# zhouxian/act3d-chained-diffuser

Measured on AMD Instinct MI355X. Metric: train samples/sec (Act3D keypose fwd+bwd+AdamW step), higher is better.
Workload: dtype fp16 / bf16 MFMA on two-part operands (x = hi + lo; fp32 accumulate) in attention; fp32-accurate linears (f32 MFMA; bf16x3 MFMA from 4096 rows); bf16 frozen backbone + FPN; 1 GPU; Act3D keypose training step, 18-PerAct-task shapes: 4 cameras 256x256, 3 ghost-point levels, 1000 ghost points (333/level), E=60, frozen synthetic CLIP-RN50-shaped backbone + trainable FPN included in the step; per_gpu_batch_keyframes=64, global_batch=64, parallelism=dp1, hipgraph=True, backbone_prefetch=True

## Files before the change

act3d-chained-diffuser_amd/csrc/conv1x1_deep.hip:

```cpp
#include "a3d_common.h"
#include "../../include/act3d_hip.h"

namespace a3d {

constexpr int CD_BM = 128, CD_BN = 128, CD_BK = 64;

__device__ __forceinline__ int cd_xoff(int row, int seg) { return row * 64 + ((seg ^ ((row >> 1) & 7)) << 3); }
__device__ __forceinline__ int cd_woff(int row, int seg) { return row * 64 + ((seg ^ ((((row >> 4) & 3) << 1) | ((row >> 1) & 1))) << 3); }

__device__ __forceinline__ unsigned int cd_norm2(unsigned int u, const float* scS, int K, int k, float relu_lo) {
  float a = __uint_as_float(u << 16) * scS[k] + scS[K + k];
  float b = __uint_as_float(u & 0xFFFF0000u) * scS[k + 1] + scS[K + k + 1];
  return pk_bf16(fmaxf(a, relu_lo), fmaxf(b, relu_lo));
}

__device__ __forceinline__ void cd_compute(const unsigned short* Xb, const unsigned short* Wb, const int (&xo)[2][4], const int (&wo)[2][4],
                                           f32x4 (&acc)[4][4]) {
#pragma unroll
  for (int h = 0; h < 2; ++h) {
    s16x8 xa[4], wb[4];
#pragma unroll
    for (int i = 0; i < 4; ++i) {
      xa[i] = *reinterpret_cast<const s16x8*>(&Xb[xo[h][i]]);
      wb[i] = *reinterpret_cast<const s16x8*>(&Wb[wo[h][i]]);
    }
#pragma unroll
    for (int tn = 0; tn < 4; ++tn)
#pragma unroll
      for (int tm = 0; tm < 4; ++tm) acc[tn][tm] = mfma_bf16_16x16x32(wb[tn], xa[tm], acc[tn][tm]);
  }
}

__device__ __forceinline__ void cd_epilogue(f32x4 (&acc)[4][4], float (&ssum)[4][4], float (&ssq)[4][4], unsigned short* __restrict__ y,
                                            long long m0, long long M, int N, int n0, int wm, int wn, int li, int g) {
#pragma unroll
  for (int tm = 0; tm < 4; ++tm) {
    const long long m = m0 + wm * 64 + tm * 16 + li;
    const bool ok = m < M;
    unsigned int pk[8];
#pragma unroll
    for (int tn = 0; tn < 4; ++tn) {
#pragma unroll
      for (int r2 = 0; r2 < 2; ++r2) {
        const unsigned int u = pk_bf16(acc[tn][tm][2 * r2], acc[tn][tm][2 * r2 + 1]);
        const float v0 = ok ? __uint_as_float(u << 16) : 0.f, v1 = ok ? __uint_as_float(u & 0xFFFF0000u) : 0.f;
        ssum[tn][2 * r2] += v0;
        ssq[tn][2 * r2] += v0 * v0;
        ssum[tn][2 * r2 + 1] += v1;
        ssq[tn][2 * r2 + 1] += v1 * v1;
        pk[2 * tn + r2] = u;
      }
      acc[tn][tm] = f32x4{0.f, 0.f, 0.f, 0.f};
    }
    if (ok) {
      uint4* dst = reinterpret_cast<uint4*>(y + (size_t)m * N + n0 + wn * 64 + g * 16);
      dst[0] = make_uint4(pk[0], pk[1], pk[2], pk[3]);
      dst[1] = make_uint4(pk[4], pk[5], pk[6], pk[7]);
    }
  }
}

template <bool XFORM>
__global__ __launch_bounds__(256, 2) void conv1x1_deep_kernel(const unsigned short* __restrict__ x, const unsigned short* __restrict__ w,
                                                            const float* __restrict__ in_scale, const float* __restrict__ in_shift,
                                                            int in_relu, unsigned short* __restrict__ y, float* __restrict__ partial,
                                                            long long M, int N, int K) {
  extern __shared__ __attribute__((aligned(16))) unsigned short smem_cd[];
  unsigned short* Xs = smem_cd;
  unsigned short* Ws = Xs + 2 * CD_BM * CD_BK;
  float* scS = reinterpret_cast<float*>(Ws + 2 * CD_BN * CD_BK);
  const int t = threadIdx.x, lane = t & 63, wave = t >> 6;
  const int li = lane & 15, g = lane >> 4;
  const int wm = wave >> 1, wn = wave & 1;
  const int n0 = blockIdx.y * CD_BN;
  const int KS = K / CD_BK;
  const long long mtiles = (M + CD_BM - 1) / CD_BM;
  if (XFORM)
    for (int i = t; i < K; i += 256) { scS[i] = in_scale[i]; scS[K + i] = in_shift[i]; }
  float ssum[4][4], ssq[4][4];
#pragma unroll
  for (int a = 0; a < 4; ++a)
#pragma unroll
    for (int r = 0; r < 4; ++r) { ssum[a][r] = 0.f; ssq[a][r] = 0.f; }
  const long long my_tiles = blockIdx.x < mtiles ? (mtiles - blockIdx.x + gridDim.x - 1) / gridDim.x : 0;
  const long long total = my_tiles * KS;
  const int srow = t >> 3, sseg = t & 7;
  long long l_m0 = (long long)blockIdx.x * CD_BM;
  int l_ks = 0;
  const float relu_lo = in_relu ? 0.f : -INFINITY;
#define CD_LOAD1(P, i)                                                                                                \
  {                                                                                                                   \
    const long long m_ = l_m0 + srow + 32 * i < M ? l_m0 + srow + 32 * i : M - 1;    \
    P##x##i = *reinterpret_cast<const uint4*>(x + (size_t)m_ * K + l_ks * CD_BK + sseg * 8);                          \
    P##w##i = *reinterpret_cast<const uint4*>(w + (size_t)(n0 + srow + 32 * i) * K + l_ks * CD_BK + sseg * 8);        \
  }
#define CD_LOAD(P)                                                                                                    \
  do {                                                                                                                \
    CD_LOAD1(P, 0) CD_LOAD1(P, 1) CD_LOAD1(P, 2) CD_LOAD1(P, 3)                                                       \
    if (l_left > 1) { --l_left; if (++l_ks == KS) { l_ks = 0; l_m0 += (long long)gridDim.x * CD_BM; } }               \
  } while (0)
#define CD_STAGE1(P, i)                                                                                               \
  {                                                                                                                   \
    uint4 v = P##x##i;                                                                                                \
    if (XFORM) {                                                                                                      \
      const int k0 = ks * CD_BK + sseg * 8;                                                                           \
      unsigned int u0 = v.x, u1 = v.y, u2 = v.z, u3 = v.w;                                                            \
      u0 = cd_norm2(u0, scS, K, k0 + 0, relu_lo); u1 = cd_norm2(u1, scS, K, k0 + 2, relu_lo);                         \
      u2 = cd_norm2(u2, scS, K, k0 + 4, relu_lo); u3 = cd_norm2(u3, scS, K, k0 + 6, relu_lo);                         \
      v = make_uint4(u0, u1, u2, u3);                                                                                 \
    }                                                                                                                 \
    *reinterpret_cast<uint4*>(&Xs[buf * CD_BM * CD_BK + cd_xoff(srow + 32 * i, sseg)]) = v;                           \
    *reinterpret_cast<uint4*>(&Ws[buf * CD_BN * CD_BK + cd_woff(srow + 32 * i, sseg)]) = P##w##i;                     \
  }
#define CD_STAGE(P) CD_STAGE1(P, 0) CD_STAGE1(P, 1) CD_STAGE1(P, 2) CD_STAGE1(P, 3)
  int xo[2][4], wo[2][4];
#pragma unroll
  for (int h = 0; h < 2; ++h)
#pragma unroll
    for (int i = 0; i < 4; ++i) {
      xo[h][i] = cd_xoff(wm * 64 + i * 16 + li, h * 4 + g);
      wo[h][i] = cd_woff(wn * 64 + (li >> 2) * 16 + i * 4 + (li & 3), h * 4 + g);
    }
  if (total > 0) {
    uint4 ax0, ax1, ax2, ax3, aw0, aw1, aw2, aw3, bx0, bx1, bx2, bx3, bw0, bw1, bw2, bw3;
    long long l_left = total;
    CD_LOAD(a);
    CD_LOAD(b);
    long long c_m0 = (long long)blockIdx.x * CD_BM;
    int ks = 0;
    f32x4 acc[4][4];
#pragma unroll
    for (int a = 0; a < 4; ++a)
#pragma unroll
      for (int b = 0; b < 4; ++b) acc[a][b] = f32x4{0.f, 0.f, 0.f, 0.f};
    __syncthreads();
#define CD_STEP(P, BUF)                                                                                               \
    {                                                                                                                 \
      constexpr int buf = BUF;                                                                                        \
      CD_STAGE(P)                                                                                                     \
      CD_LOAD(P);                                                                                \
      __syncthreads();                                             \
      cd_compute(Xs + buf * CD_BM * CD_BK, Ws + buf * CD_BN * CD_BK, xo, wo, acc);                                    \
      if (ks == KS - 1) cd_epilogue(acc, ssum, ssq, y, c_m0, M, N, n0, wm, wn, li, g);                                \
      if (++ks == KS) { ks = 0; c_m0 += (long long)gridDim.x * CD_BM; }                                               \
    }
    for (long long s = 0; s < total; s += 2) {
      CD_STEP(a, 0)
      if (s + 1 < total) CD_STEP(b, 1)
    }
#undef CD_STEP
  }
  if (!partial) return;
  __syncthreads();
  float* redS = reinterpret_cast<float*>(Xs);
  float* redQ = redS + 4 * 64;
#pragma unroll
  for (int tn = 0; tn < 4; ++tn)
#pragma unroll
    for (int r = 0; r < 4; ++r) {
      float sv = ssum[tn][r], q = ssq[tn][r];
#pragma unroll
      for (int o = 1; o < 16; o <<= 1) { sv += __shfl_xor(sv, o, 64); q += __shfl_xor(q, o, 64); }
      if (li == 0) { redS[wave * 64 + g * 16 + tn * 4 + r] = sv; redQ[wave * 64 + g * 16 + tn * 4 + r] = q; }
    }
  __syncthreads();
  if (t < CD_BN) {
    const int wn_i = t >> 6, c = t & 63;
    const float sv = redS[(0 * 2 + wn_i) * 64 + c] + redS[(1 * 2 + wn_i) * 64 + c];
    const float q = redQ[(0 * 2 + wn_i) * 64 + c] + redQ[(1 * 2 + wn_i) * 64 + c];
    float* p = partial + (size_t)blockIdx.x * 2 * N;
    p[n0 + t] = sv;
    p[N + n0 + t] = q;
  }
}

#undef CD_LOAD
#undef CD_LOAD1
#undef CD_STAGE1
#undef CD_STAGE

}

using namespace a3d;

bool a3d::conv1x1_deep_serves(int K, int N) { return K >= 128 && K <= 2048 && (K % CD_BK) == 0 && N >= 128 && N <= 2048 && (N % CD_BN) == 0; }
static size_t cd_lds(int K, bool xform) { return (size_t)2 * (CD_BM + CD_BN) * CD_BK * 2 + (xform ? (size_t)2 * K * sizeof(float) : 0); }

int a3d::conv1x1_deep_slabs(size_t M, int K, int N) {
  (void)K;
  const size_t mtiles = (M + CD_BM - 1) / CD_BM;
  const int nblocks = N / CD_BN;
  return (int)std::min<size_t>(mtiles, (size_t)std::max(1, 512 / nblocks));
}

int a3d::conv1x1_deep_launch(const void* x, const void* w, const float* in_scale, const float* in_shift, int in_relu, void* y, float* partial,
                             size_t M, int K, int N, hipStream_t s) {
  if (in_scale && K > 1024) { set_error("a3d_conv1x1_bn_fwd: the folded BatchNorm-apply of the deep-layer kernel serves K <= 1024 (K=%d)", K); return A3D_ERR_ARG; }
  static bool once = false;
  if (!once) {
    (void)hipFuncSetAttribute((const void*)conv1x1_deep_kernel<false>, hipFuncAttributeMaxDynamicSharedMemorySize, 80 * 1024);
    (void)hipFuncSetAttribute((const void*)conv1x1_deep_kernel<true>, hipFuncAttributeMaxDynamicSharedMemorySize, 80 * 1024);
    once = true;
  }
  const dim3 grid(conv1x1_deep_slabs(M, K, N), N / CD_BN);
  if (in_scale)
    hipLaunchKernelGGL(conv1x1_deep_kernel<true>, grid, dim3(256), cd_lds(K, true), s, (const unsigned short*)x, (const unsigned short*)w,
                       in_scale, in_shift, in_relu, (unsigned short*)y, partial, (long long)M, N, K);
  else
    hipLaunchKernelGGL(conv1x1_deep_kernel<false>, grid, dim3(256), cd_lds(K, false), s, (const unsigned short*)x, (const unsigned short*)w,
                       in_scale, in_shift, in_relu, (unsigned short*)y, partial, (long long)M, N, K);
  return check_launch("a3d_conv1x1_bn_fwd(deep)");
}
```

Baseline: 3476 samples/s.

## Replace deep conv1x1 kernel with 3-stage direct-to-LDS pipelined persistent GEMM

Adds a new deep-layer 1x1 conv GEMM that stages X and W tiles through a three-deep LDS ring using global_load_lds with explicit vmcnt waits, with BM selectable as 128 or 256 rows, XCD-aware persistent tile scheduling, and split partial BatchNorm-statistics output. The aim is to hide global-memory latency behind MFMA work and to improve L2 locality on MI355X. The old kernel is kept as a legacy path behind an environment variable. The change raises LDS use and drops to one workgroup per CU, and its hand-written inline asm and wait-count logic could be fragile.

```diff
diff --git a/act3d-chained-diffuser_amd/csrc/conv1x1_deep.hip b/act3d-chained-diffuser_amd/csrc/conv1x1_deep.hip
--- a/act3d-chained-diffuser_amd/csrc/conv1x1_deep.hip
+++ b/act3d-chained-diffuser_amd/csrc/conv1x1_deep.hip
@@ -1,4 +1,5 @@
 #include "a3d_common.h"
+#include "attn_ring.h"
 #include "../../include/act3d_hip.h"
 
 namespace a3d {
@@ -61,7 +62,7 @@
 }
 
 template <bool XFORM>
-__global__ __launch_bounds__(256, 2) void conv1x1_deep_kernel(const unsigned short* __restrict__ x, const unsigned short* __restrict__ w,
+__global__ __launch_bounds__(256, 2) void conv1x1_deep_legacy_kernel(const unsigned short* __restrict__ x, const unsigned short* __restrict__ w,
                                                             const float* __restrict__ in_scale, const float* __restrict__ in_shift,
                                                             int in_relu, unsigned short* __restrict__ y, float* __restrict__ partial,
                                                             long long M, int N, int K) {
@@ -179,12 +180,261 @@
 #undef CD_STAGE1
 #undef CD_STAGE
 
+
+constexpr int CR_BN = 128, CR_BK = 64, CR_STAGES = 3;
+
+template <int N_>
+__device__ __forceinline__ void cr_wait_vm() { asm volatile("s_waitcnt vmcnt(%0)" ::"n"(N_) : "memory"); }
+__device__ __forceinline__ void cr_store16(void* p, u32x4_ v) { asm volatile("global_store_dwordx4 %0, %1, off\n\ts_nop 1" ::"v"(p), "v"(v) : "memory"); }
+__device__ __forceinline__ void cr_glds16_dep(const void* g, void* lds, int& dep) {
+  const unsigned int dst = __builtin_amdgcn_readfirstlane((unsigned int)(size_t)(lds_void_t*)lds);
+  asm volatile("s_mov_b32 m0, %2\n\ts_nop 0\n\tglobal_load_lds_dwordx4 %1, off" : "+v"(dep) : "v"(g), "s"(dst) : "memory", "m0");
+}
+
+template <int TM>
+__device__ __forceinline__ void cr_compute(const unsigned short* xp0, const unsigned short* xp1, const unsigned short* wp0,
+                                           const unsigned short* wp1, f32x4 (&acc)[4][TM]) {
+#pragma unroll
+  for (int h = 0; h < 2; ++h) {
+    const unsigned short* xp = h ? xp1 : xp0;
+    const unsigned short* wp = h ? wp1 : wp0;
+    s16x8 xa[TM], wb[4];
+#pragma unroll
+    for (int i = 0; i < 4; ++i) wb[i] = *reinterpret_cast<const s16x8*>(wp + i * 4 * CR_BK);
+#pragma unroll
+    for (int i = 0; i < TM; ++i) xa[i] = *reinterpret_cast<const s16x8*>(xp + i * 16 * CR_BK);
+#pragma unroll
+    for (int tn = 0; tn < 4; ++tn)
+#pragma unroll
+      for (int tm = 0; tm < TM; ++tm) acc[tn][tm] = mfma_bf16_16x16x32(wb[tn], xa[tm], acc[tn][tm]);
+  }
+}
+
+template <int TM, bool COUNTED>
+__device__ __forceinline__ void cr_epilogue(f32x4 (&acc)[4][TM], float (&ssum)[4][4], float (&ssq)[4][4], unsigned short* __restrict__ y,
+                                            long long m0, long long M, int N, int n0, int wm, int wn, int li, int g) {
+#pragma unroll
+  for (int tm = 0; tm < TM; ++tm) {
+    const long long m = m0 + wm * (16 * TM) + tm * 16 + li;
+    const bool ok = COUNTED || m < M;
+    unsigned int pk[8];
+#pragma unroll
+    for (int tn = 0; tn < 4; ++tn) {
+#pragma unroll
+      for (int r2 = 0; r2 < 2; ++r2) {
+        const unsigned int u = pk_bf16(acc[tn][tm][2 * r2], acc[tn][tm][2 * r2 + 1]);
+        const float v0 = ok ? __uint_as_float(u << 16) : 0.f, v1 = ok ? __uint_as_float(u & 0xFFFF0000u) : 0.f;
+        ssum[tn][2 * r2] += v0;
+        ssq[tn][2 * r2] += v0 * v0;
+        ssum[tn][2 * r2 + 1] += v1;
+        ssq[tn][2 * r2 + 1] += v1 * v1;
+        pk[2 * tn + r2] = u;
+      }
+      acc[tn][tm] = f32x4{0.f, 0.f, 0.f, 0.f};
+    }
+    unsigned short* dst = y + (size_t)m * N + n0 + wn * 64 + g * 16;
+    if (COUNTED) {
+      cr_store16(dst, u32x4_{pk[0], pk[1], pk[2], pk[3]});
+      cr_store16(dst + 8, u32x4_{pk[4], pk[5], pk[6], pk[7]});
+    } else if (ok) {
+      reinterpret_cast<uint4*>(dst)[0] = make_uint4(pk[0], pk[1], pk[2], pk[3]);
+      reinterpret_cast<uint4*>(dst)[1] = make_uint4(pk[4], pk[5], pk[6], pk[7]);
+    }
+  }
+}
+
+template <bool XFORM, int TM>
+__global__ __launch_bounds__(256, 1) void conv1x1_deep_kernel(const unsigned short* __restrict__ x, const unsigned short* __restrict__ w,
+                                                            const float* __restrict__ in_scale, const float* __restrict__ in_shift,
+                                                            int in_relu, unsigned short* __restrict__ y, float* __restrict__ partial,
+                                                            long long M, int N, int K, int ngroups, int nslab) {
+  constexpr int BM = 32 * TM;
+  constexpr int STAGE = (BM + CR_BN) * CR_BK;
+  constexpr int NDMA = XFORM ? 4 : TM + 4;
+  extern __shared__ __attribute__((aligned(16))) unsigned short smem_cr[];
+  float* scS = reinterpret_cast<float*>(smem_cr + CR_STAGES * STAGE);
+  int slab, nb;
+  if (!xcd_decode(N / CR_BN, ngroups, slab, nb)) return;
+  const int t = threadIdx.x, lane = t & 63, wave = t >> 6;
+  const int li = lane & 15, g = lane >> 4;
+  const int wm = wave >> 1, wn = wave & 1;
+  const int n0 = nb * CR_BN;
+  const int KS = K / CR_BK;
+  const long long mtiles = (M + BM - 1) / BM;
+  const long long my_tiles = (mtiles - slab + ngroups - 1) / ngroups;
+  const long long total = my_tiles * KS;
+  const long long tile_stride = (long long)ngroups * BM;
+  if (XFORM) {
+    for (int i = t; i < K; i += 256) { scS[i] = in_scale[i]; scS[K + i] = in_shift[i]; }
+    __syncthreads();
+  }
+  float ssum[4][4], ssq[4][4];
+#pragma unroll
+  for (int a = 0; a < 4; ++a)
+#pragma unroll
+    for (int r = 0; r < 4; ++r) { ssum[a][r] = 0.f; ssq[a][r] = 0.f; }
+  f32x4 acc[4][TM];
+#pragma unroll
+  for (int a = 0; a < 4; ++a)
+#pragma unroll
+    for (int b = 0; b < TM; ++b) acc[a][b] = f32x4{0.f, 0.f, 0.f, 0.f};
+  const int prow = lane >> 3;
+  int xlane = XFORM ? (t & 7) << 3 : (((lane & 7) ^ (((wave & 1) << 2) | (lane >> 4))) << 3);
+  size_t wsrc[4];
+#pragma unroll
+  for (int i = 0; i < 4; ++i) {
+    const int row = (wave + 4 * i) * 8 + prow;
+    const int key = (((row >> 4) & 3) << 1) | ((row >> 1) & 1);
+    wsrc[i] = (size_t)(n0 + row) * K + (((lane & 7) ^ key) << 3);
+  }
+  const int srow = t >> 3, sseg = t & 7;
+  const float relu_lo = in_relu ? 0.f : -INFINITY;
+  long long l_m0 = (long long)slab * BM;
+  int l_ks = 0, l_st = 0;
+  long long l_left = total;
+  const unsigned short* xf0 = smem_cr + cd_xoff(wm * (16 * TM) + li, g);
+  const unsigned short* xf1 = smem_cr + cd_xoff(wm * (16 * TM) + li, 4 + g);
+  const unsigned short* wf0 = smem_cr + BM * CR_BK + cd_woff(wn * 64 + (li >> 2) * 16 + (li & 3), g);
+  const unsigned short* wf1 = smem_cr + BM * CR_BK + cd_woff(wn * 64 + (li >> 2) * 16 + (li & 3), 4 + g);
+
+#define CR_ISSUE_W()                                                                                                  \
+  {                                                                                                                   \
+    _Pragma("unroll") for (int i_ = 0; i_ < 4; ++i_)                                                                  \
+      cr_glds16_dep(w + wsrc[i_] + l_ks * CR_BK, smem_cr + l_st + BM * CR_BK + (wave + 4 * i_) * 512, xlane);         \
+  }
+#define CR_ISSUE_X()                                                                                                  \
+  {                                                                                                                   \
+    _Pragma("unroll") for (int i_ = 0; i_ < TM; ++i_) {                                                               \
+      const long long r_ = l_m0 + (wave + 4 * i_) * 8 + prow;                                                         \
+      const long long m_ = r_ < M ? r_ : M - 1;                                     \
+      glds16(x + (size_t)m_ * K + l_ks * CR_BK + xlane, smem_cr + l_st + (wave + 4 * i_) * 512);                      \
+    }                                                                                                                 \
+  }
+#define CR_LOAD_X(P)                                                                                                  \
+  {                                                                                                                   \
+    _Pragma("unroll") for (int i_ = 0; i_ < TM; ++i_) {                                                               \
+      const long long r_ = l_m0 + srow + 32 * i_;                                                                     \
+      const long long m_ = r_ < M ? r_ : M - 1;                                                                       \
+      P[i_] = *reinterpret_cast<const uint4*>(x + (size_t)m_ * K + l_ks * CR_BK + xlane);                      \
+    }                                                                                                                 \
+  }
+#define CR_ADVANCE()                                                                                                  \
+  {                                                                                                                   \
+    l_st = l_st == (CR_STAGES - 1) * STAGE ? 0 : l_st + STAGE;                                                        \
+    if (l_left > 1) { --l_left; if (++l_ks == KS) { l_ks = 0; l_m0 += tile_stride; } }    \
+  }
+#define CR_STAGE_X(P)                                                                                                 \
+  {                                                                                                                   \
+    _Pragma("unroll") for (int i_ = 0; i_ < TM; ++i_) {                                                               \
+      const int k0 = ks * CR_BK + sseg * 8;                                                                           \
+      uint4 v = P[i_];                                                                                                \
+      v = make_uint4(cd_norm2(v.x, scS, K, k0 + 0, relu_lo), cd_norm2(v.y, scS, K, k0 + 2, relu_lo),                  \
+                     cd_norm2(v.z, scS, K, k0 + 4, relu_lo), cd_norm2(v.w, scS, K, k0 + 6, relu_lo));                 \
+      *reinterpret_cast<uint4*>(&smem_cr[c_st + cd_xoff(srow + 32 * i_, sseg)]) = v;                                  \
+    }                                                                                                                 \
+  }
+  long long c_m0 = (long long)slab * BM;
+  int ks = 0, c_st = 0;
+#define CR_COMPUTE()                                                                                                  \
+  {                                                                                                                   \
+    cr_compute<TM>(xf0 + c_st, xf1 + c_st, wf0 + c_st, wf1 + c_st, acc);                                              \
+    c_st = c_st == (CR_STAGES - 1) * STAGE ? 0 : c_st + STAGE;                                                        \
+  }
+  if (XFORM) {
+    uint4 xa[TM], xb[TM];
+    CR_ISSUE_W() CR_LOAD_X(xa) CR_ADVANCE()
+    CR_ISSUE_W() CR_LOAD_X(xb) CR_ADVANCE()
+#define CR_STEP(P)                                                                                                    \
+    {                                                                                                                 \
+      CR_STAGE_X(P)                                                                                                   \
+      ring_barrier();                                              \
+      CR_ISSUE_W() CR_LOAD_X(P) CR_ADVANCE()                                                                          \
+      CR_COMPUTE()                                                                                                    \
+      if (ks == KS - 1) cr_epilogue<TM, false>(acc, ssum, ssq, y, c_m0, M, N, n0, wm, wn, li, g);                     \
+      if (++ks == KS) { ks = 0; c_m0 += tile_stride; }                                                                \
+    }
+    for (long long s = 0;;) {
+      CR_STEP(xa)
+      if (++s >= total) break;
+      CR_STEP(xb)
+      if (++s >= total) break;
+    }
+#undef CR_STEP
+    cr_wait_vm<0>();
+  } else {
+    CR_ISSUE_X() CR_ISSUE_W() CR_ADVANCE()
+    if (total > 1) { CR_ISSUE_X() CR_ISSUE_W() CR_ADVANCE() }
+    for (long long s = 0; s < total; ++s) {
+      if (s + 1 < total) {
+        if ((ks == 0 && s > 0) || (ks == 1 && s > 1)) cr_wait_vm<NDMA + 2 * TM>(); else cr_wait_vm<NDMA>();
+      } else {
+        cr_wait_vm<0>();
+      }
+      ring_barrier();
+      if (s + 2 < total) { CR_ISSUE_X() CR_ISSUE_W() CR_ADVANCE() }
+      CR_COMPUTE()
+      if (ks == KS - 1) {
+        if (c_m0 + BM <= M) cr_epilogue<TM, true>(acc, ssum, ssq, y, c_m0, M, N, n0, wm, wn, li, g);
+        else cr_epilogue<TM, false>(acc, ssum, ssq, y, c_m0, M, N, n0, wm, wn, li, g);
+      }
+      if (++ks == KS) { ks = 0; c_m0 += tile_stride; }
+    }
+  }
+#undef CR_ISSUE_W
+#undef CR_ISSUE_X
+#undef CR_LOAD_X
+#undef CR_ADVANCE
+#undef CR_STAGE_X
+#undef CR_COMPUTE
+  if (!partial) return;
+  __syncthreads();
+  float* redS = reinterpret_cast<float*>(smem_cr);
+  float* redQ = redS + 4 * 64;
+#pragma unroll
+  for (int tn = 0; tn < 4; ++tn)
+#pragma unroll
+    for (int r = 0; r < 4; ++r) {
+      float sv = ssum[tn][r], q = ssq[tn][r];
+#pragma unroll
+      for (int o = 1; o < 16; o <<= 1) { sv += __shfl_xor(sv, o, 64); q += __shfl_xor(q, o, 64); }
+      if (li == 0) { redS[wave * 64 + g * 16 + tn * 4 + r] = sv; redQ[wave * 64 + g * 16 + tn * 4 + r] = q; }
+    }
+  __syncthreads();
+  if (t < CR_BN) {
+    const int wn_i = t >> 6, c = t & 63;
+    const float s0 = redS[(0 * 2 + wn_i) * 64 + c], s1 = redS[(1 * 2 + wn_i) * 64 + c];
+    const float q0 = redQ[(0 * 2 + wn_i) * 64 + c], q1 = redQ[(1 * 2 + wn_i) * 64 + c];
+    const bool two = ngroups < nslab;
+    float* p = partial + (size_t)(two ? 2 * slab : slab) * 2 * N;
+    if (two && 2 * slab + 1 < nslab) {
+      p[n0 + t] = s0;
+      p[N + n0 + t] = q0;
+      p[2 * N + n0 + t] = s1;
+      p[3 * N + n0 + t] = q1;
+    } else {
+      p[n0 + t] = s0 + s1;
+      p[N + n0 + t] = q0 + q1;
+    }
+  }
+}
+
 }
 
 using namespace a3d;
+
+static const int cd_legacy = getenv("A3D_C1_DEEP_LEGACY") ? atoi(getenv("A3D_C1_DEEP_LEGACY")) : 0;
+static const int cd_tile = getenv("A3D_C1_DEEP_TILE") ? atoi(getenv("A3D_C1_DEEP_TILE")) : 0;
 
 bool a3d::conv1x1_deep_serves(int K, int N) { return K >= 128 && K <= 2048 && (K % CD_BK) == 0 && N >= 128 && N <= 2048 && (N % CD_BN) == 0; }
 static size_t cd_lds(int K, bool xform) { return (size_t)2 * (CD_BM + CD_BN) * CD_BK * 2 + (xform ? (size_t)2 * K * sizeof(float) : 0); }
+static size_t cr_lds(int tm, int K, bool xform) {
+  return (size_t)CR_STAGES * (32 * tm + CR_BN) * CR_BK * 2 + (xform ? (size_t)2 * K * sizeof(float) : 0);
+}
+static int cr_tm(size_t M, int N) {
+  if (cd_tile == 128) return 4;
+  if (cd_tile == 256) return 8;
+  return ((M + 255) / 256) * (size_t)(N / CR_BN) >= 256 ? 8 : 4;
+}
 
 int a3d::conv1x1_deep_slabs(size_t M, int K, int N) {
   (void)K;
@@ -193,21 +443,49 @@
   return (int)std::min<size_t>(mtiles, (size_t)std::max(1, 512 / nblocks));
 }
 
+template <bool XFORM, int TM>
+static int cr_launch(const void* x, const void* w, const float* in_scale, const float* in_shift, int in_relu, void* y, float* partial,
+                     size_t M, int K, int N, int nslab, hipStream_t s) {
+  static bool once = false;
+  if (!once) {
+    if (hipFuncSetAttribute((const void*)conv1x1_deep_kernel<XFORM, TM>, hipFuncAttributeMaxDynamicSharedMemorySize,
+                            (int)cr_lds(TM, 2048, XFORM)) != hipSuccess) {
+      (void)hipGetLastError();
+      set_error("a3d_conv1x1_bn_fwd(deep): %zu bytes of LDS per workgroup refused", cr_lds(TM, 2048, XFORM));
+      return A3D_ERR_ARG;
+    }
+    once = true;
+  }
+  const int ngroups = nslab * (N / CR_BN) <= 256 && TM == 4 ? nslab : (nslab + 1) / 2;
+  hipLaunchKernelGGL((conv1x1_deep_kernel<XFORM, TM>), dim3(xcd_grid(ngroups, N / CR_BN)), dim3(256), cr_lds(TM, K, XFORM), s,
+                     (const unsigned short*)x, (const unsigned short*)w, in_scale, in_shift, in_relu, (unsigned short*)y, partial,
+                     (long long)M, N, K, ngroups, nslab);
+  return check_launch("a3d_conv1x1_bn_fwd(deep)");
+}
+
 int a3d::conv1x1_deep_launch(const void* x, const void* w, const float* in_scale, const float* in_shift, int in_relu, void* y, float* partial,
                              size_t M, int K, int N, hipStream_t s) {
-  if (in_scale && K > 1024) { set_error("a3d_conv1x1_bn_fwd: the folded BatchNorm-apply of the deep-layer kernel serves K <= 1024 (K=%d)", K); return A3D_ERR_ARG; }
+  const int nslab = conv1x1_deep_slabs(M, K, N);
+  if (!cd_legacy) {
+    const int tm = cr_tm(M, N);
+    if (in_scale) return tm == 8 ? cr_launch<true, 8>(x, w, in_scale, in_shift, in_relu, y, partial, M, K, N, nslab, s)
+                                 : cr_launch<true, 4>(x, w, in_scale, in_shift, in_relu, y, partial, M, K, N, nslab, s);
+    return tm == 8 ? cr_launch<false, 8>(x, w, in_scale, in_shift, in_relu, y, partial, M, K, N, nslab, s)
+                   : cr_launch<false, 4>(x, w, in_scale, in_shift, in_relu, y, partial, M, K, N, nslab, s);
+  }
+  if (in_scale && K > 1024) { set_error("a3d_conv1x1_bn_fwd: the folded BatchNorm-apply of the legacy deep-layer kernel serves K <= 1024 (K=%d)", K); return A3D_ERR_ARG; }
   static bool once = false;
   if (!once) {
-    (void)hipFuncSetAttribute((const void*)conv1x1_deep_kernel<false>, hipFuncAttributeMaxDynamicSharedMemorySize, 80 * 1024);
-    (void)hipFuncSetAttribute((const void*)conv1x1_deep_kernel<true>, hipFuncAttributeMaxDynamicSharedMemorySize, 80 * 1024);
+    (void)hipFuncSetAttribute((const void*)conv1x1_deep_legacy_kernel<false>, hipFuncAttributeMaxDynamicSharedMemorySize, 80 * 1024);
+    (void)hipFuncSetAttribute((const void*)conv1x1_deep_legacy_kernel<true>, hipFuncAttributeMaxDynamicSharedMemorySize, 80 * 1024);
     once = true;
   }
-  const dim3 grid(conv1x1_deep_slabs(M, K, N), N / CD_BN);
+  const dim3 grid(nslab, N / CD_BN);
   if (in_scale)
-    hipLaunchKernelGGL(conv1x1_deep_kernel<true>, grid, dim3(256), cd_lds(K, true), s, (const unsigned short*)x, (const unsigned short*)w,
+    hipLaunchKernelGGL(conv1x1_deep_legacy_kernel<true>, grid, dim3(256), cd_lds(K, true), s, (const unsigned short*)x, (const unsigned short*)w,
                        in_scale, in_shift, in_relu, (unsigned short*)y, partial, (long long)M, N, K);
   else
-    hipLaunchKernelGGL(conv1x1_deep_kernel<false>, grid, dim3(256), cd_lds(K, false), s, (const unsigned short*)x, (const unsigned short*)w,
+    hipLaunchKernelGGL(conv1x1_deep_legacy_kernel<false>, grid, dim3(256), cd_lds(K, false), s, (const unsigned short*)x, (const unsigned short*)w,
                        in_scale, in_shift, in_relu, (unsigned short*)y, partial, (long long)M, N, K);
   return check_launch("a3d_conv1x1_bn_fwd(deep)");
 }
diff --git a/profiles/conv1x1_deep_probe.py b/profiles/conv1x1_deep_probe.py
--- /dev/null
+++ b/profiles/conv1x1_deep_probe.py
@@ -0,0 +1,59 @@
+#!/usr/bin/env python3
+import importlib
+import json
+import os
+import sys
+
+import torch
+
+sys.path.insert(0, os.path.dirname(os.path.dirname(os.path.abspath(__file__))))
+a3d = importlib.import_module("act3d-chained-diffuser_amd")
+
+SHAPES = [(262144, 128, 512, True, 3), (262144, 128, 512, False, 1), (262144, 256, 512, False, 1), (262144, 512, 128, False, 3),
+          (262144, 512, 256, False, 1), (65536, 256, 1024, True, 5), (65536, 256, 1024, False, 1), (65536, 512, 1024, False, 1),
+          (65536, 1024, 256, False, 5), (65536, 1024, 512, False, 1), (16384, 512, 2048, True, 2), (16384, 512, 2048, False, 1),
+          (16384, 1024, 2048, False, 1), (16384, 2048, 512, False, 2)]
+
+
+def main():
+    tag, out = sys.argv[1], sys.argv[2]
+    dev = torch.device("cuda:0")
+    L = a3d.lib.load()
+    res = []
+    for M, K, N, pro, n in SHAPES:
+        nbuf = max(2, -(-600_000_000 // (2 * M * (K + N))))
+        xs = [torch.randn(M, K, device=dev).to(torch.bfloat16) for _ in range(nbuf)]
+        ys = [torch.empty(M, N, device=dev, dtype=torch.bfloat16) for _ in range(nbuf)]
+        w = (torch.randn(N, K, device=dev) / K ** 0.5).to(torch.bfloat16)
+        sc = (1.0 + 0.3 * torch.randn(K, device=dev)) if pro else None
+        sh = (0.2 * torch.randn(K, device=dev)) if pro else None
+        part = torch.empty((L.a3d_conv1x1_nslab(M, K, N), 2, N), device=dev, dtype=torch.float32)
+        st = a3d.lib.stream()
+
+        def launch(i):
+            a3d.lib.call("a3d_conv1x1_bn_fwd", xs[i % nbuf].data_ptr(), w.data_ptr(), None if sc is None else sc.data_ptr(),
+                         None if sh is None else sh.data_ptr(), 1 if pro else 0, ys[i % nbuf].data_ptr(), part.data_ptr(), M, K, N, st)
+
+        for i in range(2 * nbuf):
+            launch(i)
+        torch.cuda.synchronize()
+        us = []
+        for _ in range(7):
+            e0, e1 = torch.cuda.Event(enable_timing=True), torch.cuda.Event(enable_timing=True)
+            e0.record()
+            for i in range(8):
+                launch(i)
+            e1.record()
+            torch.cuda.synchronize()
+            us.append(e0.elapsed_time(e1) * 1e3 / 8)
+        us.sort()
+        med = us[len(us) // 2]
+        res.append({"M": M, "K": K, "N": N, "prologue": pro, "n": n, "us": round(med, 1), "us_min": round(us[0], 1), "us_max": round(us[-1], 1),
+                    "PFLOPs": round(2.0 * M * K * N / med / 1e9, 3), "nslab": part.shape[0]})
+        print(tag, res[-1], flush=True)
+        del xs, ys
+    json.dump({"variant": tag, "shapes": res}, open(out, "w"))
+
+
+if __name__ == "__main__":
+    main()
```

Result: slower. 3332 samples/s (-4.2%).
